# coolbeam/UPFlow_pytorch

Measured on AMD Instinct MI355X. Metric: frame-pairs/sec at 384x1280 bf16, higher is better.
Workload: dtype bf16; 1 GPU; config2: UPFlow_net inference forward (flow fwd+bwd, occlusion masks, SGU on), 384x1280, batch 4 per GPU, random-init weights; global_batch=4, parallelism=replicas x1 (image pairs sharded, no collective), ranks=1, hip_graph=True, capture_fallback=False, steps_in_flight=4, pyramid_convs=HIP (MFMA kernel), pyramid_dtype=fp16

## Files before the change

### include/upflow_hip.h

```cpp
#ifndef UPFLOW_HIP_H
#define UPFLOW_HIP_H

#ifdef __cplusplus
extern "C" {
#endif

enum { UPF_F32 = 0, UPF_F16 = 1, UPF_BF16 = 2 };
enum { UPF_OK = 0, UPF_EINVAL = -1, UPF_EDTYPE = -2, UPF_EALIGN = -3, UPF_EUNSUPPORTED = -4 };
enum { UPF_MASK_NONE = 0, UPF_MASK_LITERAL = 1, UPF_MASK_ROBUST = 2 };

const char* upf_version(void);
const char* upf_last_error(void);

int upf_corr81_forward(const void* f1, const void* f2, void* out,
                       int B, int C, int H, int W, int dtype,
                       long long out_batch_stride, float leaky_slope, void* stream);

int upf_corr81_forward_timed(const void* f1, const void* f2, void* out,
                             int B, int C, int H, int W, int dtype,
                             long long out_batch_stride, float leaky_slope, void* stream,
                             int nrep, float* avg_us, float* min_us);

int upf_corr81_norm_supported(int C, int dtype);
long long upf_corr81_norm_workspace_bytes(int B, int C, int H, int W);
// ... 81 lines not shown

long long upf_conv_packed_bytes(int Cin, int Cout, int kernel_size);
int upf_conv_pack_weights(const void* w , void* w_packed, int Cin, int Cout, int kernel_size,
                          int dtype, void* stream);
int upf_conv_forward(const void* x, long long x_batch_stride, const void* w_packed, const float* bias,
                     void* y, long long y_batch_stride, int B, int Cin, int Cout, int H, int W,
                     int kernel_size, int dilation, int stride, float leaky_slope, int dtype, void* stream);
int upf_conv_forward_pitched(const void* x, long long x_batch_stride, int x_row_pitch, const void* w_packed, const float* bias,
                             void* y, long long y_batch_stride, int y_row_pitch, int B, int Cin, int Cout, int H, int W,
                             int kernel_size, int dilation, int stride, float leaky_slope, int dtype, void* stream);
int upf_conv1x1_forward_mixed(const void* x, long long x_batch_stride, int x_row_pitch, const void* w_packed, const float* bias,
                              void* y, long long y_batch_stride, int y_row_pitch, int y_is_c8, int B, int Cin, int Cout, int H, int W,
                              float leaky_slope, int dtype, int out_dtype, void* stream);
int upf_conv1x1_forward_c8_dual(const void* x, long long x_batch_stride, int x_row_pitch, const void* w_packed, const float* bias,
                                void* y8_a, long long ya_batch_stride, void* y8_b, long long yb_batch_stride,
                                int B, int Cin, int Cout, int H, int W, float leaky_slope, int dtype, int out_dtype, void* stream);
int upf_conv_set_option(const char* name, int value);

long long upf_conv_x3_packed_bytes(int Cin, int Cout, int kernel_size);
int upf_conv_x3_pack_weights(const float* w, void* w_packed, int Cin, int Cout, int kernel_size, void* stream);
int upf_conv_x3_forward(const float* x, long long x_batch_stride, const void* w_packed, const float* bias, float* y,
                        long long y_batch_stride, int B, int Cin, int Cout, int H, int W, int kernel_size, int dilation,
                        int stride, float leaky_slope, int nprod, void* stream);
int upf_conv_x3_set_option(const char* name, int value);
int upf_mfma_f16_denorm_probe(float* out_device, void* stream);

long long upf_conv_packed_bytes_k(int K, int Cout, int kernel_size);
int upf_conv_c8_k(int n8_oct, int C2);
int upf_conv_pack_weights_kmap(const void* w , void* w_packed, int Cin, int Cout, int kernel_size,
                               const int* kmap , int K, int dtype, void* stream);
int upf_conv_forward_c8(const void* x8, long long x8_batch_stride, int n8_oct, const void* x2, long long x2_batch_stride, int C2,
                        const void* w_packed, const float* bias, void* y, long long y_batch_stride, int y_is_c8,
                        int B, int Cout, int H, int W, int kernel_size, int dilation, int stride, float leaky_slope,
                        int dtype, void* stream);
int upf_conv_forward_c8_pitched(const void* x8, long long x8_batch_stride, int n8_oct, const void* x2, long long x2_batch_stride, int x2_row_pitch, int C2,
                                const void* w_packed, const float* bias, void* y, long long y_batch_stride, int y_row_pitch, int y_is_c8,
                                int B, int Cout, int H, int W, int kernel_size, int dilation, int stride, float leaky_slope,
                                int dtype, void* stream);
int upf_conv_c8_set_option(const char* name, int value);
long long upf_conv_packed_bytes_k16(int K, int Cout);
int upf_conv_pack_weights_kmap16(const void* w , void* w_packed, int Cin, int Cout,
                                 const int* kmap , int K, int dtype, void* stream);
int upf_conv_forward_c8_narrow(const void* x8, long long x8_batch_stride, int n8_oct, const void* w_packed16, const float* bias,
                               void* y, long long y_batch_stride, int y_is_c8, int B, int Cout, int H, int W, float leaky_slope,
                               int dtype, void* stream);
int upf_conv_forward_c8_split(const void* x8, long long x8_batch_stride, int n8_oct, const void* w_packed ,
                              const float* bias , void* y8, long long y_batch_stride, int C_main,
                              float* partial, long long partial_batch_stride , int partial_pitch ,
                              int B, int Cout, int H, int W, float leaky_slope, int dtype, void* stream);
int upf_conv_forward_c8_narrow_init(const void* x8, long long x8_batch_stride, int n8_oct, const void* w_packed16,
                                    const float* partial, long long partial_batch_stride, int partial_pitch, int partial_offset ,
                                    void* y, long long y_batch_stride, int y_is_c8, int B, int Cout, int H, int W, float leaky_slope,
                                    int dtype, void* stream);

int upf_conv_pair_forward(const void* x, long long x_batch_stride, int x_row_pitch, int Cin,
                          const void* wa_packed, const float* bias_a , float slope_a, int C1, int stride_a,
                          const void* wb_packed, const float* bias_b , float slope_b, int C2, int stride_b,
                          void* y, long long y_batch_stride, int y_row_pitch, int y_is_c8,
                          int B, int H, int W, int dtype, void* stream);

int upf_conv_pack_weights_f32(const float* w , void* w_packed, int Cin, int Cout, int kernel_size,
                              int dtype, int dgrad, void* stream);
int upf_conv_pack_weights_f32_multi(const float* const* w, void* const* w_packed, const int* Cin, const int* Cout, const int* kernel_size,
                                    const int* dgrad, int njobs, int dtype, void* stream);
int upf_conv_pack_stacked_dgrad(const float* const* w, const int* Cin, const int* Cout, const int* first_channel, int nlayers,
                                void* const* w_packed, const int* slice_channel, const int* slice_width, const int* nconsumers,
                                int nslices, int dtype, void* stream);
int upf_leaky_backward(const void* grad_y, const void* y, void* grad_pre, long long n, float slope, int dtype, void* stream);
int upf_conv_wgrad_supported(int Cin, int Cout, int H, int W, int kernel_size, int dilation, int stride, int dtype);
long long upf_conv_wgrad_workspace_bytes(int B, int Cin, int Cout, int H, int W, int kernel_size, int dilation);
int upf_conv_wgrad(const void* x, long long x_batch_stride, const void* grad_pre, long long g_batch_stride, float* grad_w,
                   void* workspace, int B, int Cin, int Cout, int H, int W, int kernel_size, int dilation, int dtype, void* stream);
typedef struct {
  const void* x;        long long x_batch_stride;
  const void* grad_pre; long long g_batch_stride;
  int B, H, W;
} upf_wgrad_level;
long long upf_conv_wgrad_multi_workspace_bytes(const upf_wgrad_level* levels, int nlevels, int Cin, int Cout, int kernel_size, int dilation);
int upf_conv_wgrad_multi(const upf_wgrad_level* levels , int nlevels, float* grad_w, void* workspace, int Cin, int Cout,
                         int kernel_size, int dilation, int dtype, void* stream);
int upf_conv_wgrad_multi_bias(const upf_wgrad_level* levels, int nlevels, float* grad_w, void* workspace, int Cin, int Cout,
                              int kernel_size, int dilation, const float* const* bias_partials , int npartials, float* grad_bias,
                              int dtype, void* stream);
int upf_space_to_depth2(const void* src, void* dst, int B, int C , int H, int W , int inverse, int dtype, void* stream);
int upf_conv_wgrad_s2d(const upf_wgrad_level* levels, int nlevels, float* grad_w, void* workspace, int Cin, int Cout, int dtype, void* stream);
int upf_act_grad(const void* src, long long src_batch_stride, const void* add, long long add_batch_stride, const void* y,
                 long long y_batch_stride, void* dst, long long dst_batch_stride, float* bias_partial, int B, int C, int HW,
                 float slope, int dtype, void* stream);
int upf_conv_forward_gated(const void* x, long long x_batch_stride, int x_row_pitch, const void* w_packed, const float* bias,
                           void* y, long long y_batch_stride, int y_row_pitch, const void* add, long long add_batch_stride,
                           const void* act, long long act_batch_stride, float mask_slope,
                           int B, int Cin, int Cout, int H, int W, int dtype, void* stream);
int upf_conv_bias_grad_finish(const float* const* partials , int npartials, float* grad_bias,
                              int Cout, void* stream);
long long upf_conv_bias_grad_workspace_bytes(int Cout);
int upf_conv_bias_grad(const void* grad_pre, long long g_batch_stride, float* grad_bias, void* workspace, int B, int Cout, int HW,
                       int dtype, void* stream);

int upf_act_grad_x3(const float* grad_y, long long gy_batch_stride, const float* y, long long y_batch_stride, float* grad_pre_scaled,
                    long long dst_batch_stride, float* bias_partial, float* scale_slot, int B, int C, int HW, float slope, void* stream);
int upf_conv_x3_pack_weights_dgrad(const float* w, void* w_packed, int Cin, int Cout, int kernel_size, void* stream);
int upf_conv_x3_dgrad(const float* grad_pre_scaled, long long g_batch_stride, const float* scale_slot, const float* w,
                      void* w_packed_dgrad, const float* zero_bias, float* grad_x, long long gx_batch_stride, int B, int Cin,
                      int Cout, int H, int W, int kernel_size, int dilation, int stride, void* stream);
int upf_conv_x3_wgrad_workspace_bytes(const upf_wgrad_level* levels, int nlevels, int Cin, int Cout, int kernel_size,
                                      int dilation, int stride, long long* bytes );
// ... 49 lines not shown
```

### upflow_pytorch_amd/_build.py

```python
import os
import subprocess
import sys

PKG = os.path.dirname(os.path.abspath(__file__))
CSRC = os.path.join(PKG, 'csrc')
LIB = os.path.join(PKG, 'libupflow_hip.so')

SOURCES = [
    ('api.hip', []),
    ('corr81_fwd.hip', ['-ffp-contract=off']),
    ('corr81_bwd.hip', []),
    ('conv3x3.hip', []),
    ('conv_c8.hip', []),
    ('conv_pair.hip', []),
    ('conv_x3.hip', []),
    ('conv_x3_bwd.hip', []),
    ('conv_wgrad.hip', []),
    ('warp.hip', ['-ffp-contract=off']),
    ('sgu_blend.hip', ['-ffp-contract=off']),
    ('misc.hip', ['-ffp-contract=off']),
    ('loss.hip', ['-ffp-contract=off']),
]
COMMON = ['--offload-arch=gfx950', '-O3', '-std=c++17', '-fPIC', '-fno-gpu-rdc', '-Wall', '-Wno-unused-function']
NO_PACKED_FP32 = ['-Xclang', '-target-feature', '-Xclang', '-packed-fp32-ops']


def hipcc():
    for c in (os.environ.get('HIPCC'), '/opt/rocm/bin/hipcc', 'hipcc'):
        if c and (os.path.isabs(c) and os.path.exists(c) or not os.path.isabs(c)):
            return c
    raise RuntimeError('hipcc not found')


def _stale(target, deps):
    if not os.path.exists(target):
        return True
    t = os.path.getmtime(target)
    return any(os.path.getmtime(d) > t for d in deps)


def _flags_tag(extra):
    import hashlib
    return hashlib.sha256(' '.join(COMMON + NO_PACKED_FP32 + list(extra)).encode()).hexdigest()[:16]


def _flags_stale(obj, extra):
    try:
        return open(obj + '.flags').read().strip() != _flags_tag(extra)
    except OSError:
        return True


def build(force=False, verbose=False):
    headers = [os.path.join(CSRC, h) for h in os.listdir(CSRC) if h.endswith('.hpp')]
    headers.append(os.path.join(os.path.dirname(PKG), 'include', 'upflow_hip.h'))
    objdir = os.path.join(PKG, 'build')
    os.makedirs(objdir, exist_ok=True)
    objs = []
    cc = hipcc()
    jobs = []
    for src, extra in SOURCES:
        s = os.path.join(CSRC, src)
        o = os.path.join(objdir, src.replace('.hip', '.o'))
        objs.append(o)
        if force or _stale(o, [s] + headers) or _flags_stale(o, extra):
            jobs.append(([cc] + COMMON + NO_PACKED_FP32 + extra + ['-c', s, '-o', o], o, extra))

# ... 29 lines not shown
```

### upflow_pytorch_amd/_lib.py

```python
import ctypes
import os

import torch

_PKG = os.path.dirname(os.path.abspath(__file__))
LIB_PATH = os.environ.get('UPF_HIP_LIB') or os.path.join(_PKG, 'libupflow_hip.so')

UPF_F32, UPF_F16, UPF_BF16 = 0, 1, 2
MASK_NONE, MASK_LITERAL, MASK_ROBUST = 0, 1, 2
_DTYPES = {torch.float32: UPF_F32, torch.float16: UPF_F16, torch.bfloat16: UPF_BF16}

_c = ctypes
_vp, _i, _f, _ll = _c.c_void_p, _c.c_int, _c.c_float, _c.c_longlong

SIGNATURES = {
    'upf_corr81_forward': [_vp, _vp, _vp, _i, _i, _i, _i, _i, _ll, _f, _vp],
    'upf_corr81_forward_timed': [_vp, _vp, _vp, _i, _i, _i, _i, _i, _ll, _f, _vp, _i, _c.POINTER(_f), _c.POINTER(_f)],
    'upf_corr81_norm_forward': [_vp, _vp, _vp, _i, _i, _i, _i, _i, _ll, _f, _vp, _vp],
    'upf_corr81_norm_forward_timed': [_vp, _vp, _vp, _i, _i, _i, _i, _i, _ll, _f, _vp, _vp, _i, _c.POINTER(_f), _c.POINTER(_f)],
    'upf_corr81_norm_forward_c8_timed': [_vp, _vp, _vp, _ll, _i, _i, _i, _i, _i, _f, _vp, _vp, _i, _c.POINTER(_f), _c.POINTER(_f)],
    'upf_corr81_norm_forward_pitched': [_vp, _vp, _i, _vp, _i, _i, _i, _i, _i, _ll, _f, _vp, _vp],
    'upf_corr81_norm_forward_c8_pitched': [_vp, _vp, _i, _vp, _ll, _i, _i, _i, _i, _i, _f, _vp, _vp],
    'upf_corr81_norm_forward_c8_timed_pitched': [_vp, _vp, _i, _vp, _ll, _i, _i, _i, _i, _i, _f, _vp, _vp, _i, _c.POINTER(_f), _c.POINTER(_f)],
    'upf_corr81_norm_forward_c8_timed_mixed': [_vp, _vp, _i, _vp, _ll, _i, _i, _i, _i, _i, _i, _f, _vp, _vp, _i, _c.POINTER(_f), _c.POINTER(_f)],
    'upf_warp_forward_pitched': [_vp, _ll, _i, _vp, _vp, _ll, _i, _i, _i, _i, _i, _i, _i, _i, _vp],
    'upf_conv_forward_gated': [_vp, _ll, _i, _vp, _vp, _vp, _ll, _i, _vp, _ll, _vp, _ll, _f, _i, _i, _i, _i, _i, _i, _vp],
    'upf_conv_forward_pitched': [_vp, _ll, _i, _vp, _vp, _vp, _ll, _i, _i, _i, _i, _i, _i, _i, _i, _i, _f, _i, _vp],
    'upf_conv_forward_c8_pitched': [_vp, _ll, _i, _vp, _ll, _i, _i, _vp, _vp, _vp, _ll, _i, _i, _i, _i, _i, _i, _i, _i, _i, _f, _i, _vp],
    'upf_corr81_norm_forward_mixed': [_vp, _vp, _i, _vp, _i, _i, _i, _i, _i, _i, _ll, _f, _vp, _vp],
    'upf_corr81_norm_forward_c8_mixed': [_vp, _vp, _i, _vp, _ll, _i, _i, _i, _i, _i, _i, _f, _vp, _vp],
    'upf_conv1x1_forward_mixed': [_vp, _ll, _i, _vp, _vp, _vp, _ll, _i, _i, _i, _i, _i, _i, _i, _f, _i, _i, _vp],
    'upf_conv1x1_forward_c8_dual': [_vp, _ll, _i, _vp, _vp, _vp, _ll, _vp, _ll, _i, _i, _i, _i, _i, _f, _i, _i, _vp],
    'upf_corr81_backward': [_vp, _vp, _vp, _vp, _vp, _i, _i, _i, _i, _i, _vp],
    'upf_correlation_forward': [_vp, _vp, _vp, _i, _i, _i, _i, _i, _i, _i, _i, _i, _i, _i, _vp],
    'upf_correlation_backward': [_vp, _vp, _vp, _vp, _vp, _i, _i, _i, _i, _i, _i, _i, _i, _i, _i, _i, _vp],
    'upf_correlation_out_shape': [_i, _i, _i, _i, _i, _i, _i, _c.POINTER(_i), _c.POINTER(_i), _c.POINTER(_i)],
    'upf_warp_forward': [_vp, _vp, _vp, _i, _i, _i, _i, _i, _i, _i, _vp],
    'upf_warp_forward_strided': [_vp, _ll, _vp, _vp, _ll, _i, _i, _i, _i, _i, _i, _i, _vp],
    'upf_warp_forward_c8': [_vp, _ll, _vp, _vp, _ll, _i, _i, _i, _i, _i, _i, _i, _vp],
    'upf_flow_update': [_vp, _vp, _vp, _vp, _ll, _i, _i, _i, _i, _vp],
    'upf_flow_update_c8': [_vp, _vp, _vp, _vp, _ll, _i, _i, _i, _vp],
    'upf_corr81_norm_forward_c8': [_vp, _vp, _vp, _ll, _i, _i, _i, _i, _i, _f, _vp, _vp],
    'upf_warp_backward': [_vp, _vp, _vp, _vp, _vp, _vp, _i, _i, _i, _i, _i, _i, _i, _vp],
    'upf_flow_upsample_forward': [_vp, _vp, _i, _i, _i, _i, _i, _i, _i, _vp],
    'upf_flow_upsample_backward': [_vp, _vp, _i, _i, _i, _i, _i, _i, _i, _vp],
    'upf_sgu_blend_forward': [_vp, _vp, _vp, _vp, _vp, _vp, _i, _i, _i, _i, _i, _i, _vp],
    'upf_sgu_blend_forward_flow16': [_vp, _vp, _vp, _vp, _ll, _i, _i, _i, _i, _i, _vp],
    'upf_sgu_blend_backward': [_vp, _vp, _vp, _vp, _vp, _vp, _i, _i, _i, _i, _i, _i, _vp],
    'upf_normalize_forward': [_vp, _vp, _vp, _vp, _vp, _ll, _i, _i, _vp],
    'upf_normalize_backward': [_vp, _vp, _vp, _vp, _ll, _i, _i, _vp],
    'upf_conv_pack_weights': [_vp, _vp, _i, _i, _i, _i, _vp],
    'upf_conv_forward': [_vp, _ll, _vp, _vp, _vp, _ll, _i, _i, _i, _i, _i, _i, _i, _i, _f, _i, _vp],
    'upf_conv_x3_pack_weights': [_vp, _vp, _i, _i, _i, _vp],
    'upf_conv_x3_forward': [_vp, _ll, _vp, _vp, _vp, _ll, _i, _i, _i, _i, _i, _i, _i, _i, _f, _i, _vp],
    'upf_mfma_f16_denorm_probe': [_vp, _vp],
    'upf_act_grad_x3': [_vp, _ll, _vp, _ll, _vp, _ll, _vp, _vp, _i, _i, _i, _f, _vp],
    'upf_conv_x3_pack_weights_dgrad': [_vp, _vp, _i, _i, _i, _vp],
    'upf_conv_x3_dgrad': [_vp, _ll, _vp, _vp, _vp, _vp, _vp, _ll, _i, _i, _i, _i, _i, _i, _i, _i, _vp],
    'upf_conv_x3_wgrad_workspace_bytes': [_vp, _i, _i, _i, _i, _i, _i, _c.POINTER(_ll)],
    'upf_conv_x3_wgrad': [_vp, _vp, _i, _vp, _vp, _i, _i, _i, _i, _i, _vp, _vp, _vp],
    'upf_conv_pack_weights_f32': [_vp, _vp, _i, _i, _i, _i, _i, _vp],
    'upf_conv_pack_stacked_dgrad': [_c.POINTER(_vp), _c.POINTER(_i), _c.POINTER(_i), _c.POINTER(_i), _i, _c.POINTER(_vp), _c.POINTER(_i), _c.POINTER(_i), _c.POINTER(_i), _i, _i, _vp],
    'upf_conv_pack_weights_f32_multi': [_c.POINTER(_vp), _c.POINTER(_vp), _c.POINTER(_i), _c.POINTER(_i), _c.POINTER(_i), _c.POINTER(_i), _i, _i, _vp],
    'upf_conv_pack_weights_kmap': [_vp, _vp, _i, _i, _i, _vp, _i, _i, _vp],
    'upf_conv_forward_c8': [_vp, _ll, _i, _vp, _ll, _i, _vp, _vp, _vp, _ll, _i, _i, _i, _i, _i, _i, _i, _i, _f, _i, _vp],
    'upf_conv_pack_weights_kmap16': [_vp, _vp, _i, _i, _vp, _i, _i, _vp],
    'upf_conv_forward_c8_narrow': [_vp, _ll, _i, _vp, _vp, _vp, _ll, _i, _i, _i, _i, _i, _f, _i, _vp],
    'upf_conv_forward_c8_split': [_vp, _ll, _i, _vp, _vp, _vp, _ll, _i, _vp, _ll, _i, _i, _i, _i, _i, _f, _i, _vp],
    'upf_conv_forward_c8_narrow_init': [_vp, _ll, _i, _vp, _vp, _ll, _i, _i, _vp, _ll, _i, _i, _i, _i, _i, _f, _i, _vp],
    'upf_conv_pair_forward': [_vp, _ll, _i, _i, _vp, _vp, _f, _i, _i, _vp, _vp, _f, _i, _i, _vp, _ll, _i, _i, _i, _i, _i, _i, _vp],
    'upf_leaky_backward': [_vp, _vp, _vp, _ll, _f, _i, _vp],
    'upf_conv_wgrad': [_vp, _ll, _vp, _ll, _vp, _vp, _i, _i, _i, _i, _i, _i, _i, _i, _vp],
    'upf_conv_bias_grad': [_vp, _ll, _vp, _vp, _i, _i, _i, _i, _vp],
    'upf_conv_wgrad_multi': [_vp, _i, _vp, _vp, _i, _i, _i, _i, _i, _vp],
    'upf_conv_wgrad_multi_bias': [_vp, _i, _vp, _vp, _i, _i, _i, _i, _vp, _i, _vp, _i, _vp],
    'upf_space_to_depth2': [_vp, _vp, _i, _i, _i, _i, _i, _i, _vp],
    'upf_conv_wgrad_s2d': [_vp, _i, _vp, _vp, _i, _i, _i, _vp],
    'upf_act_grad': [_vp, _ll, _vp, _ll, _vp, _ll, _vp, _ll, _vp, _i, _i, _i, _f, _i, _vp],
    'upf_conv_bias_grad_finish': [_vp, _i, _vp, _i, _vp],
    'upf_census_forward': [_vp, _vp, _vp, _i, _i, _i, _i, _vp],
    'upf_census_backward': [_vp, _vp, _vp, _vp, _vp, _i, _i, _i, _i, _vp],
    'upf_boundary_warp_forward': [_vp, _vp, _vp, _vp, _i, _i, _i, _i, _i, _i, _vp],
    'upf_boundary_warp_backward': [_vp, _vp, _vp, _vp, _vp, _i, _i, _i, _i, _i, _i, _vp],
    'upf_robust_loss_forward': [_vp, _vp, _vp, _vp, _i, _i, _i, _f, _f, _vp],
    'upf_robust_loss_backward': [_vp, _vp, _vp, _vp, _vp, _vp, _i, _i, _i, _f, _f, _vp],
    'upf_grey_forward': [_vp, _vp, _i, _i, _vp],
    'upf_msd_upup_forward': [_vp, _vp, _vp, _i, _vp, _vp, _vp, _vp, _i, _i, _i, _f, _f, _f, _vp],
    'upf_msd_upup_backward': [_vp, _vp, _vp, _vp, _i, _vp, _vp, _vp, _vp, _i, _i, _i, _f, _f, _f, _vp],
    'upf_smooth_edge1_forward': [_vp, _vp, _vp, _i, _i, _i, _i, _i, _vp],
    'upf_smooth_edge1_backward': [_vp, _vp, _vp, _vp, _i, _i, _i, _i, _i, _vp],
    'upf_div_selftest': [_i, _vp, _vp],
    'upf_occ_check': [_vp, _vp, _vp, _vp, _i, _i, _i, _f, _f, _vp],
}



class WgradLevel(_c.Structure):
    _fields_ = [('x', _vp), ('x_batch_stride', _ll), ('grad_pre', _vp), ('g_batch_stride', _ll), ('B', _i), ('H', _i), ('W', _i)]


_lib = None


class UpflowHipError(RuntimeError):
    """Raised for a rejected argument or a failed launch (the reference raises RuntimeError through
    AT_ERROR("CUDA call failed"), correlation_cuda.cc:81-83)."""


def lib():
    global _lib
    if _lib is None:
        if not os.path.exists(LIB_PATH):
            raise UpflowHipError(
                '%s is missing: build it with `python -c "import __graft_entry__ as g; g.build()"` '
                '(hipcc --offload-arch=gfx950). There is no CPU fallback.' % LIB_PATH)
        L = ctypes.CDLL(LIB_PATH)
        for name, argtypes in SIGNATURES.items():
            fn = getattr(L, name)
            fn.argtypes = argtypes
            fn.restype = _i
        L.upf_normalize_workspace_bytes.argtypes = [_ll, _i]
        L.upf_normalize_workspace_bytes.restype = _ll
# ... 91 lines not shown
```

### upflow_pytorch_amd/model/pwc_modules.py

```python
import logging

import torch
import torch.nn as nn
import torch.nn.functional as tf

from .. import ops
from ..utils.tools import tools


def conv(in_planes, out_planes, kernel_size=3, stride=1, dilation=1, isReLU=True, if_IN=False, IN_affine=False, if_BN=False):
    layers = [nn.Conv2d(in_planes, out_planes, kernel_size=kernel_size, stride=stride, dilation=dilation,
                        padding=((kernel_size - 1) * dilation) // 2, bias=True)]
    if isReLU:
        layers.append(nn.LeakyReLU(0.1, inplace=True))
    if if_IN:
        layers.append(nn.InstanceNorm2d(out_planes, affine=IN_affine))
    elif if_BN:
        layers.append(nn.BatchNorm2d(out_planes, affine=IN_affine))
    return nn.Sequential(*layers)


def initialize_msra(modules):
    logging.info("Initializing MSRA")
    for layer in modules:
        if isinstance(layer, (nn.Conv2d, nn.ConvTranspose2d)):
            nn.init.kaiming_normal_(layer.weight)
            if layer.bias is not None:
                nn.init.constant_(layer.bias, 0)


def upsample2d_as(inputs, target_as, mode="bilinear"):
    _, _, h, w = target_as.size()
    return tf.interpolate(inputs, [h, w], mode=mode, align_corners=True)


def _resize_flow(inputs, h, w, mode, if_rate):
    if mode != "bilinear":
        res = tf.interpolate(inputs, [h, w], mode=mode)
        if if_rate:
            _, _, h_, w_ = inputs.size()
            scale = torch.tensor([w / w_, h / h_], dtype=res.dtype, device=res.device).view(1, 2, 1, 1)
            res = res * scale
        return res
    return ops.flow_upsample(inputs, h, w, if_rate)


def upsample2d_flow_as(inputs, target_as, mode="bilinear", if_rate=False):
    _, _, h, w = target_as.size()
    return _resize_flow(inputs, h, w, mode, if_rate)


def upsample_flow(inputs, target_size=None, target_flow=None, mode="bilinear"):
    if target_size is not None:
# ... 231 lines not shown
                J.append(j); used += need
            if not J or any(widths[k] % 8 for k in range(m, n - 1)):
                continue
            score = len(J) * (cin[m] + 1000)
            if score > best_score:
                best, best_score = (m, sorted(J)), score
        return best

    def _key(self):
        k = []
        for c in self.convs:
            k += [c.weight._version, c.weight.dtype, c.weight.device, c.weight.data_ptr(), c.bias._version, c.bias.data_ptr()]
        return tuple(k)

    def get(self):
        key = self._key()
        if key != self.key:
            c0 = self.main
            rows, bias = [c0.weight.detach()], [c0.bias.detach().float()]
            self.finish = {}
            for j, c in zip(self.J, self.convs[1:]):
                front = sum(self.widths[self.m:j])
                w = c.weight.detach()
                assert w.shape[1] == front + self.cin
                pad = (c.out_channels + 3) // 4 * 4 - c.out_channels
                rows.append(w[:, front:])
                bias.append(c.bias.detach().float())
                if pad:
                    rows.append(w.new_zeros((pad, self.cin) + tuple(w.shape[2:])))
                    bias.append(bias[0].new_zeros(pad))
                self.finish[j] = ops.conv_c8_pack16(w[:, :front].contiguous(), list(range(front)))
            self.packed = ops.conv_c8_pack(torch.cat(rows, 0).contiguous(), self.kmap)
            self.bias = torch.cat(bias).contiguous()
            self.key = key
        return self.packed, self.bias

    def extra_operands(self):
        return list(self.finish.values())

    def invalidate(self):
        self.key = None

    def main_pass(self, x8, y8):
        packed, bias = self.get()
        B, _, H, W, _ = x8.shape
        part = torch.empty((B, self.pp // 4, H, W, 4), dtype=torch.float32, device=x8.device)
        ops.conv_c8_forward_split_raw(x8, packed, bias, y8, part, self.slopes[self.m])
        return part

    def finish_pass(self, j, x8_front, part, y):
        self.get()
        return ops.conv_c8_forward_narrow_init_raw(x8_front, self.finish[j], part, self.offsets[j], self.widths[j], y, self.slopes[j])


class _PackedConvPair(object):

    def __init__(self, seq_a, seq_b):
        self.convs = (seq_a[0], seq_b[0])
        self.strides = (seq_a[0].stride[0], seq_b[0].stride[0])
        self.slopes = tuple(0.1 if any(isinstance(m_, nn.LeakyReLU) for m_ in q) else 0.0 for q in (seq_a, seq_b))
        self.key = None
        self.packed = self.packed_b = self.bias = self.bias_b = None

    def _key(self):
        k = []
        for c in self.convs:
            k += [c.weight._version, c.weight.dtype, c.weight.device, c.weight.data_ptr(), c.bias._version, c.bias.data_ptr()]
        return tuple(k)

    def get(self):
        key = self._key()
        if key != self.key:
            a, b = self.convs
            self.packed, self.packed_b = ops.conv_pair_pack(a.weight, b.weight)
            self.bias, self.bias_b = a.bias.detach().float().contiguous(), b.bias.detach().float().contiguous()
            self.key = key
        return self.packed, self.bias, self.packed_b, self.bias_b

    def extra_operands(self):
        return [self.packed_b, self.bias_b]

    def invalidate(self):
        self.key = None

    def __call__(self, x, y):
        pa, ba, pb, bb = self.get()
        return ops.conv_pair_forward_raw(x, pa, ba, self.slopes[0], pb, bb, self.slopes[1], y, self.strides)


DUAL_1X1 = [True]
FUSE_PAIRS = [True]
MERGE_TAIL = [True]


def c8_level_ok(nb, H, W, dtype):
    return dtype in (torch.bfloat16, torch.float16) and nb * ((W + 31) // 32) * ((H + 7) // 8) >= 200


def fast_conv_seq(seq, x, cache, out=None, allow_hip=True, pitched=False):
    c = seq[0]
    k = c.kernel_size[0]
    if (allow_hip and _fast_conv_ok(x) and c.kernel_size in ((3, 3), (1, 1)) and c.stride[0] == c.stride[1] and c.groups == 1 and len(seq) <= 2
            and c.padding == (((k - 1) * c.dilation[0]) // 2,) * 2
            and (ops.conv3x3_supported(x, c.out_channels, c.dilation[0], c.stride[0], k)
                 or (x.shape[3] < 8 and 1 <= c.dilation[0] <= 16 and (c.stride[0] == 1 or (c.stride[0] == 2 and c.dilation[0] == 1 and k == 3))))):
        pc = cache.get(id(seq))
        if pc is None:
            pc = cache[id(seq)] = _PackedConv3x3(seq)
        ho, wo = ops.conv3x3_out_hw(x.shape[2], x.shape[3], c.stride[0])
        y = out if out is not None else ops.empty_nchw((x.shape[0], c.out_channels, ho, wo), x.dtype, x.device, pitched=pitched)
        return pc(x, y)
    if torch.is_grad_enabled() and x.is_cuda and x.dtype in (torch.bfloat16, torch.float16) and c.weight.dtype == torch.float32:
        y = train_conv_seq(seq, x)
    elif (FP32_TRAIN_CONV[0] == 'hip_x3' and torch.is_grad_enabled() and x.is_cuda and x.dtype == torch.float32
          and c.weight.dtype == torch.float32):
        y = train_conv_seq_x3(seq, x)
    else:
        y = seq(x if x.is_contiguous() else x.contiguous())
    if out is not None:
        out.copy_(y)
        return out
    return y


def train_conv_seq(seq, x):
    c = seq[0]
    k = c.kernel_size[0]
    slope = 0.0
    for m in list(seq)[1:]:
        if isinstance(m, nn.LeakyReLU):
            slope = float(m.negative_slope)
        else:
            return seq(x.float()).to(x.dtype)
    if (c.kernel_size in ((3, 3), (1, 1)) and c.stride[0] == c.stride[1] and c.groups == 1 and c.padding == (((k - 1) * c.dilation[0]) // 2,) * 2
            and ops.conv_train_supported(x, c.weight, c.stride[0], c.dilation[0])):
        return ops.conv_train(x, c.weight, c.bias, c.dilation[0], slope, c.stride[0])
    return seq(x.float()).to(x.dtype)


def train_conv_seq_x3(seq, x):
    c = seq[0]
    k = c.kernel_size[0]
    slope = 0.0
    for m in list(seq)[1:]:
        if not isinstance(m, nn.LeakyReLU):
# ... 69 lines not shown
        return buf, buf[:, x0:self._n_total]

    def forward_in_buffer(self, buf, out=None):
        if self._packed is None:
            self._packed = [_PackedConv3x3(getattr(self, n)) for n in self._NAMES] + [_PackedConv3x3(self.conv_last)]
        nt = self._n_total
        hi = nt - self._ch_in
        for pc, f in zip(self._packed[:5], self._f):
            pc(buf[:, hi:nt], buf[:, hi - f:hi])
            hi -= f
        x5 = buf[:, :nt]
        if out is None:
            out = torch.empty((buf.shape[0], self.conv_last[0].out_channels) + tuple(buf.shape[2:]), dtype=buf.dtype, device=buf.device)
        self._packed[5](x5, out)
        return x5, out

    def c8_ok(self):
        return self._ch_in % 8 == 0 and all(f % 8 == 0 for f in self._f)

    def c8_outputs_ok(self):
        return all(f % 8 == 0 for f in self._f)

    def forward_in_buffer_c8(self, buf8, out=None, in_map=None):
        key = None if in_map is None else tuple(in_map)
        cache = self.__dict__.setdefault('_packed8', {})
        if key not in cache:
            imap = list(range(self._ch_in)) if in_map is None else list(in_map)
            assert len(imap) % 8 == 0 and sorted(m for m in imap if m >= 0) == list(range(self._ch_in)), 'in_map must place every input channel once'
            packed, nconv = [], 0
            for name, f in zip(self._NAMES, self._f):
                packed.append(_PackedConvC8(getattr(self, name), list(range(nconv)) + [m + nconv if m >= 0 else -1 for m in imap]))
                nconv += f
            packed.append(_PackedConvC8(self.conv_last, list(range(nconv)) + [m + nconv if m >= 0 else -1 for m in imap]))
            widths = list(self._f) + [self.conv_last[0].out_channels]
            seqs = [getattr(self, n_) for n_ in self._NAMES] + [self.conv_last]
            plain = all(all(isinstance(x_, (nn.Conv2d, nn.LeakyReLU)) for x_ in q_) for q_ in seqs)
            pl = _PackedTailC8.plan(widths) if plain else None
            if pl is not None:
                nbefore = sum(self._f[:pl[0]])
                packed.append(_PackedTailC8(seqs, pl[0], pl[1], list(range(nbefore)) + [q + nbefore if q >= 0 else -1 for q in imap]))
            cache[key] = (packed, len(imap) // 8)
        packed, n_in = cache[key]
        nl = len(self._f)
        no = sum(self._f) // 8 + n_in
        starts, hi = [], sum(self._f) // 8
        for f in self._f:
            starts.append(hi)
            hi -= f // 8
        starts.append(hi)
        if out is None:
            out = torch.empty((buf8.shape[0], self.conv_last[0].out_channels) + tuple(buf8.shape[2:4]), dtype=buf8.dtype, device=buf8.device)
        tail = packed[nl + 1] if (len(packed) > nl + 1 and MERGE_TAIL[0] and not getattr(self, '_no_merge_tail', False)) else None
        part = None
        for k in range(nl + 1):
            y = buf8[:, starts[k + 1]:starts[k]] if k < nl else out
            if tail is not None and k == tail.m:
                part = tail.main_pass(buf8[:, starts[k]:no], y)
            elif tail is not None and k in tail.J:
                tail.finish_pass(k, buf8[:, starts[k]:starts[tail.m]], part, y)
            else:
                packed[k](buf8[:, starts[k]:no], None, y)
        return out

    def _train_convs(self):
        seqs = [getattr(self, n) for n in self._NAMES] + [self.conv_last]
        slope = None
        for i, q in enumerate(seqs):
            act = list(q)[1:]
            if i < 5:
                if len(act) != 1 or not isinstance(act[0], nn.LeakyReLU):
                    return None, None
                slope = float(act[0].negative_slope)
            elif act:
                return None, None
        return [q[0] for q in seqs], slope

    def train_in_buffer_ok(self, inputs):
        convs, _ = self._train_convs()
        return convs is not None and not getattr(self, '_no_train_buffer', False) and ops.dense_stack_train_supported(inputs, convs)

    def forward_train(self, inputs, flow_tail=None):
        convs, slope = self._train_convs()
        return ops.dense_stack_train(inputs, convs, slope, flow_tail)

    def forward(self, x):
        if _fast_conv_ok(x):
            buf, slot = self.alloc_buffer(x.shape[0], x.shape[2], x.shape[3], x.dtype, x.device)
            slot.copy_(x)
            return self.forward_in_buffer(buf)
        if self.train_in_buffer_ok([x]):
            buf, out = self.forward_train([x])
            return buf, out
        cache = self.__dict__.setdefault('_fast_cache', {})
        for name in self._NAMES:
            x = torch.cat([fast_conv_seq(getattr(self, name), x, cache), x], dim=1)
        return x, fast_conv_seq(self.conv_last, x, cache)


class FlowEstimatorDense_v2(_DenseStack):
    def __init__(self, ch_in, f_channels=(128, 128, 96, 64, 32), out_channel=2):
        super(FlowEstimatorDense_v2, self).__init__()
        self.n_channels = self._build(ch_in, f_channels, out_channel)


class FlowEstimatorDense(FlowEstimatorDense_v2):

    def __init__(self, ch_in):
        super(FlowEstimatorDense, self).__init__(ch_in)


# ... 51 lines not shown
```

### upflow_pytorch_amd/ops.py

```python
import os

import torch
from torch.autograd import Function

from . import _lib
from ._operand_cache import OperandCache
from ._lib import MASK_NONE, MASK_LITERAL, MASK_ROBUST, UpflowHipError

_MASKS = {None: MASK_NONE, 'none': MASK_NONE, 'literal': MASK_LITERAL, 'robust': MASK_ROBUST,
          MASK_NONE: MASK_NONE, MASK_LITERAL: MASK_LITERAL, MASK_ROBUST: MASK_ROBUST}


def _f32(t):
    return t if t.dtype == torch.float32 else t.float()


PITCH_MULTIPLE = 8


def empty_nchw(shape, dtype, device, pitched=True):
    W = shape[-1]
    if pitched and dtype in (torch.bfloat16, torch.float16) and W >= 8 and W % PITCH_MULTIPLE:
        Wp = (W + PITCH_MULTIPLE - 1) // PITCH_MULTIPLE * PITCH_MULTIPLE
        return torch.empty(tuple(shape[:-1]) + (Wp,), dtype=dtype, device=device)[..., :W]
# ... 746 lines not shown
        if not _c8_view_ok(y) or tuple(y.shape) != (B, (Cout + 7) // 8, H, W, 8):
            raise UpflowHipError('conv_c8_narrow: C8 output must be [%d,%d,%d,%d,8], got %s' % (B, (Cout + 7) // 8, H, W, tuple(y.shape)))
    elif tuple(y.shape) != (B, Cout, H, W) or y.stride()[1:] != (H * W, W, 1):
        raise UpflowHipError('conv_c8_narrow: NCHW output must be a [%d,%d,%d,%d] channel slice' % (B, Cout, H, W))
    dev = x8.device
    if not (x8.is_cuda and y.is_cuda) or x8.dtype != y.dtype:
        raise UpflowHipError('conv_c8_narrow: GPU tensors of one dtype expected (there is no CPU fallback)')
    with torch.cuda.device(dev):
        _lib.call('upf_conv_forward_c8_narrow', _lib.ptr(x8), x8.stride(0), n, _lib.ptr(packed16), _lib.ptr(bias32), _lib.ptr(y), y.stride(0),
                  int(y_is_c8), B, Cout, H, W, float(leaky_slope), _lib.dtype_code(x8), _lib.stream_ptr(dev))
    return y


def _partial_ok(partial, B, H, W):
    return (partial.dtype == torch.float32 and partial.dim() == 5 and partial.shape[0] == B and tuple(partial.shape[2:]) == (H, W, 4)
            and partial.stride()[1:] == (H * W * 4, W * 4, 4, 1))


def conv_c8_forward_split_raw(x8, packed, bias32, y8, partial, leaky_slope=0.0):
    B, n, H, W, _ = x8.shape
    Cout = bias32.shape[0]
    if not _c8_view_ok(x8) or not _c8_view_ok(y8) or tuple(y8.shape[0:1] + y8.shape[2:]) != (B, H, W, 8):
        raise UpflowHipError('conv_c8_split: x8 / y8 must be octet slices of contiguous C8 buffers of one size')
    cmain = 8 * y8.shape[1]
    if not _partial_ok(partial, B, H, W) or 4 * partial.shape[1] < (Cout - cmain + 3) // 4 * 4:
        raise UpflowHipError('conv_c8_split: partial must be fp32 [B,Q,H,W,4] (planes of channel quads, 4 Q >= the partial channels), got %s' % (tuple(partial.shape),))
    dev = x8.device
    if not (x8.is_cuda and y8.is_cuda and partial.is_cuda) or x8.dtype != y8.dtype:
        raise UpflowHipError('conv_c8_split: GPU tensors of one 16-bit dtype expected (there is no CPU fallback)')
    with torch.cuda.device(dev):
        _lib.call('upf_conv_forward_c8_split', _lib.ptr(x8), x8.stride(0), n, _lib.ptr(packed), _lib.ptr(bias32), _lib.ptr(y8), y8.stride(0), cmain,
                  _lib.ptr(partial), partial.stride(0), 4 * partial.shape[1], B, Cout, H, W, float(leaky_slope), _lib.dtype_code(x8), _lib.stream_ptr(dev))
    return y8


def conv_c8_forward_narrow_init_raw(x8, packed16, partial, offset, Cout, y, leaky_slope=0.0):
    B, n, H, W, _ = x8.shape
    y_is_c8 = y.dim() == 5
    if not _c8_view_ok(x8):
        raise UpflowHipError('conv_c8_narrow_init: x8 must be an octet slice of a contiguous C8 buffer')
    if y_is_c8:
        if not _c8_view_ok(y) or tuple(y.shape) != (B, (Cout + 7) // 8, H, W, 8):
            raise UpflowHipError('conv_c8_narrow_init: C8 output must be [%d,%d,%d,%d,8], got %s' % (B, (Cout + 7) // 8, H, W, tuple(y.shape)))
    elif tuple(y.shape) != (B, Cout, H, W) or y.stride()[1:] != (H * W, W, 1):
        raise UpflowHipError('conv_c8_narrow_init: NCHW output must be a [%d,%d,%d,%d] channel slice' % (B, Cout, H, W))
    if not _partial_ok(partial, B, H, W):
        raise UpflowHipError('conv_c8_narrow_init: partial must be fp32 [B,Q,H,W,4] (planes of channel quads)')
    dev = x8.device
    if not (x8.is_cuda and y.is_cuda and partial.is_cuda) or x8.dtype != y.dtype:
        raise UpflowHipError('conv_c8_narrow_init: GPU tensors of one 16-bit dtype expected (there is no CPU fallback)')
    with torch.cuda.device(dev):
        _lib.call('upf_conv_forward_c8_narrow_init', _lib.ptr(x8), x8.stride(0), n, _lib.ptr(packed16), _lib.ptr(partial), partial.stride(0), 4 * partial.shape[1],
                  int(offset), _lib.ptr(y), y.stride(0), int(y_is_c8), B, int(Cout), H, W, float(leaky_slope), _lib.dtype_code(x8), _lib.stream_ptr(dev))
    return y


def conv_pair_pack(w_a, w_b):
    C1, Cin, C2 = w_a.shape[0], w_a.shape[1], w_b.shape[0]
    if tuple(w_a.shape[2:]) != (3, 3) or tuple(w_b.shape[2:]) != (3, 3) or w_b.shape[1] != C1 or Cin > 16 or C1 not in (16, 32) or C2 > 32:
        raise UpflowHipError('conv_pair_pack: 3x3 layers with Cin <= 16, C1 = 16 | 32, C2 <= 32 expected, got %s / %s' % (tuple(w_a.shape), tuple(w_b.shape)))
    dev, dt = w_a.device, w_a.dtype
    lane = torch.arange(64, device=dev)
    co, kg, j = (lane % 32).view(1, 64, 1), (lane // 32).view(1, 64, 1), torch.arange(8, device=dev).view(1, 1, 8)
    wa = torch.zeros((32, 16, 12), dtype=dt, device=dev)
    wa[:C1, :Cin, :9] = w_a.detach().reshape(C1, Cin, 9)
    if Cin <= 4:
        s = torch.arange(3, device=dev).view(3, 1, 1)
        pa = wa[co.expand(3, 64, 8), (j % 4).expand(3, 64, 8), (4 * s + 2 * kg + j // 4).expand(3, 64, 8)]
    elif Cin <= 8:
        s = torch.arange(5, device=dev).view(5, 1, 1)
        pa = wa[co.expand(5, 64, 8), j.expand(5, 64, 8), (2 * s + kg).expand(5, 64, 8)]
    else:
        s = torch.arange(9, device=dev).view(9, 1, 1)
        pa = wa[co.expand(9, 64, 8), (8 * kg + j).expand(9, 64, 8), s.expand(9, 64, 8)]
    ksb = C1 // 16
    wbz = torch.zeros((32, C1, 9), dtype=dt, device=dev)
    wbz[:C2] = w_b.detach().reshape(C2, C1, 9)
    tap = torch.arange(9, device=dev).view(9, 1, 1, 1)
    ks = torch.arange(ksb, device=dev).view(1, ksb, 1, 1)
    shp = (9, ksb, 64, 8)
    pb = wbz[co.view(1, 1, 64, 1).expand(shp), (16 * ks + 8 * kg.view(1, 1, 64, 1) + j.view(1, 1, 1, 8)).expand(shp), tap.expand(shp)]
    return pa.contiguous(), pb.contiguous()


def conv_pair_forward_raw(x, packed_a, bias_a, slope_a, packed_b, bias_b, slope_b, y, strides=(1, 2)):
    B, Cin, H, W = x.shape
    C1, C2 = bias_a.shape[0], bias_b.shape[0]
    Ho, Wo = conv3x3_out_hw(H, W, 2)
    xp = _pitch_or_raise(x, 'conv_pair: x')
    y_is_c8 = y.dim() == 5
    if y_is_c8:
        if not _c8_view_ok(y) or tuple(y.shape) != (B, (C2 + 7) // 8, Ho, Wo, 8):
            raise UpflowHipError('conv_pair: C8 output must be [%d,%d,%d,%d,8], got %s' % (B, (C2 + 7) // 8, Ho, Wo, tuple(y.shape)))
        yp = 0
    else:
        if tuple(y.shape) != (B, C2, Ho, Wo):
            raise UpflowHipError('conv_pair: NCHW output must be [%d,%d,%d,%d], got %s' % (B, C2, Ho, Wo, tuple(y.shape)))
        yp = _out_pitch_or_raise(y, 'conv_pair: y')
    dev = x.device
    if not (x.is_cuda and y.is_cuda) or x.dtype != y.dtype or x.dtype not in (torch.bfloat16, torch.float16) or packed_a.dtype != x.dtype:
        raise UpflowHipError('conv_pair: GPU tensors of one 16-bit dtype expected (there is no CPU fallback)')
    with torch.cuda.device(dev):
        _lib.call('upf_conv_pair_forward', _lib.ptr(x), x.stride(0), xp, Cin, _lib.ptr(packed_a), _lib.ptr(bias_a), float(slope_a), C1, int(strides[0]),
                  _lib.ptr(packed_b), _lib.ptr(bias_b), float(slope_b), C2, int(strides[1]), _lib.ptr(y), y.stride(0), yp, int(y_is_c8), B, H, W,
                  _lib.dtype_code(x), _lib.stream_ptr(dev))
    return y
# ... 1074 lines not shown
```

Baseline: 1943 frame-pairs/s.

## Fuse last two narrow tail convolutions into one kernel with LDS halo recompute

Adds a HIP kernel that runs the final 16->8 conv and the last 8->Cout conv of the dense-net tail in one launch. The intermediate 8-channel activation is computed with a one-pixel halo into LDS and consumed directly by the second conv, while still being written to the C8 buffer. The goal is to save one kernel launch and the global round trip of the middle activation, at the cost of recomputing the halo and using more LDS per block. It is enabled by default when the layer widths match and can be turned off with an environment variable.

```diff
diff --git a/include/upflow_hip.h b/include/upflow_hip.h
--- a/include/upflow_hip.h
+++ b/include/upflow_hip.h
@@ -157,6 +157,10 @@
                                     const float* partial, long long partial_batch_stride, int partial_pitch, int partial_offset ,
                                     void* y, long long y_batch_stride, int y_is_c8, int B, int Cout, int H, int W, float leaky_slope,
                                     int dtype, void* stream);
+int upf_conv_forward_c8_tail2(const void* x8, long long x8_batch_stride, int n8_oct, const void* w_packed16_a, const void* w_packed16_b,
+                              const float* partial, long long partial_batch_stride, int partial_pitch, int partial_offset_a, int partial_offset_b,
+                              void* y_mid8, long long y_mid_batch_stride, int C_mid, void* y, long long y_batch_stride,
+                              int B, int Cout, int H, int W, float leaky_slope_a, float leaky_slope_b, int dtype, void* stream);
 
 int upf_conv_pair_forward(const void* x, long long x_batch_stride, int x_row_pitch, int Cin,
                           const void* wa_packed, const float* bias_a , float slope_a, int C1, int stride_a,
diff --git a/upflow_pytorch_amd/_build.py b/upflow_pytorch_amd/_build.py
--- a/upflow_pytorch_amd/_build.py
+++ b/upflow_pytorch_amd/_build.py
@@ -13,6 +13,7 @@
     ('conv3x3.hip', []),
     ('conv_c8.hip', []),
     ('conv_pair.hip', []),
+    ('conv_tail2.hip', []),
     ('conv_x3.hip', []),
     ('conv_x3_bwd.hip', []),
     ('conv_wgrad.hip', []),
diff --git a/upflow_pytorch_amd/_lib.py b/upflow_pytorch_amd/_lib.py
--- a/upflow_pytorch_amd/_lib.py
+++ b/upflow_pytorch_amd/_lib.py
@@ -68,6 +68,7 @@
     'upf_conv_forward_c8_narrow': [_vp, _ll, _i, _vp, _vp, _vp, _ll, _i, _i, _i, _i, _i, _f, _i, _vp],
     'upf_conv_forward_c8_split': [_vp, _ll, _i, _vp, _vp, _vp, _ll, _i, _vp, _ll, _i, _i, _i, _i, _i, _f, _i, _vp],
     'upf_conv_forward_c8_narrow_init': [_vp, _ll, _i, _vp, _vp, _ll, _i, _i, _vp, _ll, _i, _i, _i, _i, _i, _f, _i, _vp],
+    'upf_conv_forward_c8_tail2': [_vp, _ll, _i, _vp, _vp, _vp, _ll, _i, _i, _i, _vp, _ll, _i, _vp, _ll, _i, _i, _i, _i, _f, _f, _i, _vp],
     'upf_conv_pair_forward': [_vp, _ll, _i, _i, _vp, _vp, _f, _i, _i, _vp, _vp, _f, _i, _i, _vp, _ll, _i, _i, _i, _i, _i, _i, _vp],
     'upf_leaky_backward': [_vp, _vp, _vp, _ll, _f, _i, _vp],
     'upf_conv_wgrad': [_vp, _ll, _vp, _ll, _vp, _vp, _i, _i, _i, _i, _i, _i, _i, _i, _vp],
diff --git a/upflow_pytorch_amd/csrc/conv_tail2.hip b/upflow_pytorch_amd/csrc/conv_tail2.hip
--- /dev/null
+++ b/upflow_pytorch_amd/csrc/conv_tail2.hip
@@ -0,0 +1,212 @@
+#include "conv_kernel.hpp"
+
+namespace upf {
+namespace conv {
+
+struct Tail2Part { const float* part; long long pbs; int ppitch, coffa, coffb; };
+
+template <typename T, int RPW>
+__global__ __launch_bounds__(NTHREADS, 4)
+void conv_tail2_sgu_kernel(const T* __restrict__ x8, long long x8bs, const T* __restrict__ wpa, const T* __restrict__ wpb,
+                           T* __restrict__ ymid, long long ymbs, T* __restrict__ y, long long ybs, int CoutB, int H, int W,
+                           int tiles_x, int tiles_y, float slope_a, float slope_b, const Tail2Part pa) {
+  constexpr int TH = 4 * RPW;
+  constexpr int XR = TH + 4, XC = TW + 4, XP = XC | 1;
+  constexpr int MR = TH + 2, MC = TW + 2, MP = MC | 1;
+  constexpr int EB = 2 * XR * XP, EBP = (EB + 63) & ~63, NSL = (EBP / 64 + 3) / 4;
+  constexpr int NPX = MR * MC, NG = (NPX + 15) / 16, NGW = (NG + 3) / 4;
+  extern __shared__ __attribute__((aligned(16))) uint4 xs[];
+  uint4* mid = xs + EBP;
+
+  const int bid = xcd_remap(blockIdx.x, gridDim.x);
+  const int tx = bid % tiles_x, ty = (bid / tiles_x) % tiles_y, n = bid / (tiles_x * tiles_y);
+  const int x0 = tx * TW, y0 = ty * TH;
+  const int tid = threadIdx.x, lane = tid & 63;
+  const int wave_u = __builtin_amdgcn_readfirstlane(tid >> 6);
+  const int p16 = lane & 15, ko = lane >> 4;
+  const int HW = H * W;
+
+  __amdgpu_buffer_rsrc_t x8r = __builtin_amdgcn_make_buffer_rsrc(const_cast<T*>(x8 + (size_t)n * x8bs), 0, 2u * (uint32_t)HW * 16u, 0x00020000);
+#pragma unroll
+  for (int j = 0; j < NSL; ++j) {
+    const int piece = j * 4 + wave_u;
+    if (piece * 64 < EBP) {
+      const int p = piece * 64 + lane;
+      const int oct = p / (XR * XP), rem = p - oct * (XR * XP), r = rem / XP, col = rem - r * XP;
+      const int gy = y0 - 2 + r, gx = x0 - 2 + col;
+      const bool in = p < EB && col < XC && gy >= 0 && gy < H && gx >= 0 && gx < W;
+      const uint32_t voff = in ? (uint32_t)((oct * HW + gy * W + gx) * 16) : 0x80000000u;
+      __builtin_amdgcn_raw_ptr_buffer_load_lds(x8r, (__attribute__((address_space(3))) void*)(xs + piece * 64), 16, (int)voff, 0, 0, 0);
+    }
+  }
+
+  __amdgpu_buffer_rsrc_t pr = __builtin_amdgcn_make_buffer_rsrc(const_cast<float*>(pa.part + (size_t)n * pa.pbs), 0, (uint32_t)HW * (uint32_t)pa.ppitch * 4u, 0x00020000);
+  f32x4 acca[NGW];
+#pragma unroll
+  for (int i = 0; i < NGW; ++i) {
+    const int q = (wave_u + 4 * i) * 16 + p16, qq = q < NPX ? q : 0;
+    const int mr = qq / MC, mc = qq - mr * MC, gy = y0 - 1 + mr, gx = x0 - 1 + mc;
+    const bool in = q < NPX && gy >= 0 && gy < H && gx >= 0 && gx < W && ko < 2;
+    const uint32_t off = in ? (uint32_t)(((pa.coffa >> 2) + ko) * HW + gy * W + gx) * 16u : 0x80000000u;
+    acca[i] = __builtin_bit_cast(f32x4, __builtin_amdgcn_raw_buffer_load_b128(pr, off, 0, 0));
+  }
+
+  uint4 wa[9];
+#pragma unroll
+  for (int tap = 0; tap < 9; ++tap) wa[tap] = reinterpret_cast<const uint4*>(wpa)[tap * 64 + lane];
+
+  asm volatile("s_waitcnt vmcnt(0)" ::: "memory");
+  __syncthreads();
+
+  __amdgpu_buffer_rsrc_t mr_ = __builtin_amdgcn_make_buffer_rsrc(ymid + (size_t)n * ymbs, 0, (uint32_t)HW * 16u, 0x00020000);
+  __builtin_amdgcn_s_setprio(2);
+#pragma unroll
+  for (int i = 0; i < NGW; ++i) {
+    if (wave_u + 4 * i < NG) {
+      const int q = (wave_u + 4 * i) * 16 + p16, qq = q < NPX ? q : 0;
+      const int mr = qq / MC, mc = qq - mr * MC, gy = y0 - 1 + mr, gx = x0 - 1 + mc;
+      const bool in = q < NPX && gy >= 0 && gy < H && gx >= 0 && gx < W;
+      const uint4* xb = xs + ((ko & 1) * XR + mr) * XP + mc;
+      uint4 b[9];
+#pragma unroll
+      for (int tap = 0; tap < 9; ++tap) {
+        b[tap] = xb[(tap / 3) * XP + tap % 3];
+        if (ko >= 2) b[tap] = make_uint4(0u, 0u, 0u, 0u);
+      }
+      f32x4 acc = acca[i];
+#pragma unroll
+      for (int tap = 0; tap < 9; ++tap) acc = Mma16<T>::mma(wa[tap], b[tap], acc);
+      float v[4];
+#pragma unroll
+      for (int k = 0; k < 4; ++k) { v[k] = acc[k]; v[k] = fmaxf(v[k], v[k] * slope_a); }
+      u32x2 o;
+      o.x = pack2<T>(v[0], v[1]); o.y = pack2<T>(v[2], v[3]);
+      if (!in) { o.x = 0u; o.y = 0u; }
+      if (q < NPX && ko < 2) reinterpret_cast<u32x2*>(mid)[(mr * MP + mc) * 2 + ko] = o;
+      const bool own = in && ko < 2 && mr >= 1 && mr <= TH && mc >= 1 && mc <= TW;
+      __builtin_amdgcn_raw_buffer_store_b64(o, mr_, own ? (uint32_t)(gy * W + gx) * 16u + (uint32_t)ko * 8u : 0x80000000u, 0, 0);
+    }
+  }
+  __builtin_amdgcn_s_setprio(0);
+  const int rg = wave_u;
+  f32x4 accb[RPW][2];
+#pragma unroll
+  for (int r = 0; r < RPW; ++r)
+#pragma unroll
+    for (int h = 0; h < 2; ++h) {
+      const int gx = x0 + p16 + 16 * h, gy = y0 + RPW * rg + r;
+      const uint32_t off = (gx < W && gy < H && 4 * ko < CoutB) ? (uint32_t)(((pa.coffb >> 2) + ko) * HW + gy * W + gx) * 16u : 0x80000000u;
+      accb[r][h] = __builtin_bit_cast(f32x4, __builtin_amdgcn_raw_buffer_load_b128(pr, off, 0, 0));
+    }
+  uint4 wb[9];
+#pragma unroll
+  for (int tap = 0; tap < 9; ++tap) wb[tap] = reinterpret_cast<const uint4*>(wpb)[tap * 64 + lane];
+  __syncthreads();
+
+  constexpr int NR = RPW + 2;
+  const uint4* bb = ko == 0 ? mid + (RPW * rg) * MP + p16 : xs + (((ko - 1) & 1) * XR + RPW * rg + 1) * XP + p16 + 1;
+  const int bp = ko == 0 ? MP : XP;
+  uint4 bq[2][6];
+  auto bload = [&](int sr, uint4 (&b)[6]) {
+#pragma unroll
+    for (int h = 0; h < 2; ++h)
+#pragma unroll
+      for (int kx = 0; kx < 3; ++kx) {
+        b[h * 3 + kx] = bb[sr * bp + 16 * h + kx];
+        if (ko == 3) b[h * 3 + kx] = make_uint4(0u, 0u, 0u, 0u);
+      }
+  };
+  __builtin_amdgcn_s_setprio(2);
+  bload(0, bq[0]);
+#pragma unroll
+  for (int sr = 0; sr < NR; ++sr) {
+    if (sr + 1 < NR) bload(sr + 1, bq[(sr + 1) & 1]);
+    __builtin_amdgcn_sched_barrier(0);
+#pragma unroll
+    for (int kx = 0; kx < 3; ++kx)
+#pragma unroll
+      for (int h = 0; h < 2; ++h)
+#pragma unroll
+        for (int ky = 0; ky < 3; ++ky)
+          if (sr - ky >= 0 && sr - ky < RPW)
+            accb[sr - ky][h] = Mma16<T>::mma(wb[ky * 3 + kx], bq[sr & 1][h * 3 + kx], accb[sr - ky][h]);
+    __builtin_amdgcn_sched_barrier(0);
+  }
+  __builtin_amdgcn_s_setprio(0);
+
+  const uint32_t plane2 = (uint32_t)HW * 2u;
+  __amdgpu_buffer_rsrc_t yr = __builtin_amdgcn_make_buffer_rsrc(y + (size_t)n * ybs, 0, (uint32_t)CoutB * plane2, 0x00020000);
+#pragma unroll
+  for (int r = 0; r < RPW; ++r) {
+    const int gy = y0 + RPW * rg + r;
+    if (gy < H) {
+#pragma unroll
+      for (int h = 0; h < 2; ++h) {
+        const int gx = x0 + p16 + 16 * h;
+        float v[4];
+#pragma unroll
+        for (int k = 0; k < 4; ++k) { v[k] = accb[r][h][k]; v[k] = fmaxf(v[k], v[k] * slope_b); }
+        const uint32_t off = (gx < W) ? (uint32_t)(4 * ko) * plane2 + (uint32_t)(gy * W + gx) * 2u : 0x80000000u;
+        const uint32_t p01 = pack2<T>(v[0], v[1]), p23 = pack2<T>(v[2], v[3]);
+        __builtin_amdgcn_raw_buffer_store_b16((unsigned short)p01, yr, off, 0, 0);
+        __builtin_amdgcn_raw_buffer_store_b16((unsigned short)(p01 >> 16), yr, off + plane2, 0, 0);
+        __builtin_amdgcn_raw_buffer_store_b16((unsigned short)p23, yr, off + 2u * plane2, 0, 0);
+        __builtin_amdgcn_raw_buffer_store_b16((unsigned short)(p23 >> 16), yr, off + 3u * plane2, 0, 0);
+      }
+    }
+  }
+}
+
+struct ArgsTail2 {
+  const void* x8; long long x8bs; const void* wpa; const void* wpb; void* ymid; long long ymbs; void* y; long long ybs;
+  int B, CoutB, H, W; float slope_a, slope_b; hipStream_t stream;
+};
+
+template <typename T, int RPW>
+int launch_tail2_sgu(const ArgsTail2& a, const Tail2Part& pa) {
+  constexpr int TH = 4 * RPW;
+  constexpr int EB = 2 * (TH + 4) * ((TW + 4) | 1), EBP = (EB + 63) & ~63;
+  const int tiles_x = cdiv(a.W, TW), tiles_y = cdiv(a.H, TH);
+  const size_t lds = (size_t)(EBP + (TH + 2) * ((TW + 2) | 1)) * 16;
+  static LdsOptIn opt;
+  auto kern = &conv_tail2_sgu_kernel<T, RPW>;
+  opt.ensure(reinterpret_cast<const void*>(kern), lds);
+  hipLaunchKernelGGL(kern, dim3((unsigned)(a.B * tiles_x * tiles_y)), dim3(NTHREADS), lds, a.stream, (const T*)a.x8, a.x8bs, (const T*)a.wpa, (const T*)a.wpb,
+                     (T*)a.ymid, a.ymbs, (T*)a.y, a.ybs, a.CoutB, a.H, a.W, tiles_x, tiles_y, a.slope_a, a.slope_b, pa);
+  return check_launch("conv_forward_c8_tail2");
+}
+
+
+}
+}
+
+extern "C" int upf_conv_forward_c8_tail2(const void* x8, long long x8_batch_stride, int n8_oct, const void* w_packed16_a, const void* w_packed16_b,
+                                         const float* partial, long long partial_batch_stride, int partial_pitch, int partial_offset_a, int partial_offset_b,
+                                         void* y_mid8, long long y_mid_batch_stride, int C_mid, void* y, long long y_batch_stride,
+                                         int B, int Cout, int H, int W, float leaky_slope_a, float leaky_slope_b, int dtype, void* stream) {
+  using namespace upf;
+  UPF_REQUIRE(x8 && w_packed16_a && w_packed16_b && partial && y_mid8 && y, UPF_EINVAL, "conv_forward_c8_tail2: null pointer");
+  UPF_REQUIRE(n8_oct == 2 && C_mid == 8, UPF_EUNSUPPORTED, "conv_forward_c8_tail2: a 16 -> 8 first layer only (got %d octets -> %d channels)", n8_oct, C_mid);
+  UPF_REQUIRE(B > 0 && Cout > 0 && Cout <= 16 && H > 0 && W > 0, UPF_EINVAL, "conv_forward_c8_tail2: bad shape B=%d Cout=%d (<= 16) H=%d W=%d", B, Cout, H, W);
+  UPF_REQUIRE(partial_pitch % 4 == 0 && partial_offset_a % 4 == 0 && partial_offset_a >= 0 && partial_offset_a + C_mid <= partial_pitch &&
+              partial_offset_b % 4 == 0 && partial_offset_b >= 0 && partial_offset_b + (Cout + 3) / 4 * 4 <= partial_pitch, UPF_EINVAL,
+              "conv_forward_c8_tail2: partial pitch %d / offsets %d, %d must be multiples of 4 floats holding the layers' %d and %d channels",
+              partial_pitch, partial_offset_a, partial_offset_b, C_mid, Cout);
+  UPF_REQUIRE(dtype == UPF_BF16 || dtype == UPF_F16, UPF_EDTYPE, "conv_forward_c8_tail2: bf16 / fp16 only");
+  UPF_REQUIRE(aligned_to(x8, 16) && x8_batch_stride % 8 == 0 && aligned_to(partial, 16) && partial_batch_stride % 4 == 0, UPF_EINVAL,
+              "conv_forward_c8_tail2: the C8 input and the partial must be 16-byte aligned");
+  UPF_REQUIRE(aligned_to(y_mid8, 16) && y_mid_batch_stride % 8 == 0, UPF_EINVAL, "conv_forward_c8_tail2: the C8 output must be 16-byte aligned");
+  UPF_REQUIRE(aligned_to(w_packed16_a, 16) && aligned_to(w_packed16_b, 16), UPF_EINVAL, "conv_forward_c8_tail2: the packed operands must be 16-byte aligned");
+  UPF_REQUIRE((long long)n8_oct * H * W * 16 < (1ll << 31) && (long long)H * W * partial_pitch * 4 < (1ll << 31), UPF_EINVAL,
+              "conv_forward_c8_tail2: image too large for one buffer descriptor");
+  UPF_REQUIRE((long long)Cout * H * W * 2 < (1ll << 31), UPF_EINVAL, "conv_forward_c8_tail2: output too large for one buffer descriptor");
+  UPF_REQUIRE(leaky_slope_a >= 0.f && leaky_slope_a <= 1.f && leaky_slope_b >= 0.f && leaky_slope_b <= 1.f, UPF_EINVAL,
+              "conv_forward_c8_tail2: leaky slopes %g, %g not in [0,1]", (double)leaky_slope_a, (double)leaky_slope_b);
+  const conv::ArgsTail2 a{x8, x8_batch_stride, w_packed16_a, w_packed16_b, y_mid8, y_mid_batch_stride, y, y_batch_stride, B, Cout, H, W,
+                          leaky_slope_a == 0.f ? 1.f : leaky_slope_a, leaky_slope_b == 0.f ? 1.f : leaky_slope_b, (hipStream_t)stream};
+  const conv::Tail2Part pa{partial, partial_batch_stride, partial_pitch, partial_offset_a, partial_offset_b};
+#define UPF_TAIL2(T) return conv::launch_tail2_sgu<T, 2>(a, pa);
+  if (dtype == UPF_BF16) { UPF_TAIL2(bf16_t) }
+  UPF_TAIL2(f16_t)
+#undef UPF_TAIL2
+}
diff --git a/upflow_pytorch_amd/model/pwc_modules.py b/upflow_pytorch_amd/model/pwc_modules.py
--- a/upflow_pytorch_amd/model/pwc_modules.py
+++ b/upflow_pytorch_amd/model/pwc_modules.py
@@ -1,4 +1,5 @@
 import logging
+import os
 
 import torch
 import torch.nn as nn
@@ -336,6 +337,17 @@
         self.get()
         return ops.conv_c8_forward_narrow_init_raw(x8_front, self.finish[j], part, self.offsets[j], self.widths[j], y, self.slopes[j])
 
+    def pair_ok(self):
+        n = len(self.widths)
+        return (self.J == [n - 2, n - 1] and self.m == n - 3
+                and ops.conv_c8_tail2_supported(self.widths[self.m], self.widths[n - 2], self.widths[n - 1]))
+
+    def finish_pair(self, x8_main, part, y_mid8, y):
+        self.get()
+        ja, jb = self.J
+        return ops.conv_c8_forward_tail2_raw(x8_main, self.finish[ja], self.finish[jb], part, self.offsets[ja], self.offsets[jb], y_mid8,
+                                             self.widths[jb], y, self.slopes[ja], self.slopes[jb])
+
 
 class _PackedConvPair(object):
 
@@ -375,6 +387,7 @@
 DUAL_1X1 = [True]
 FUSE_PAIRS = [True]
 MERGE_TAIL = [True]
+FUSE_TAIL2 = [not os.environ.get('UPF_NO_FUSE_TAIL2')]
 
 
 def c8_level_ok(nb, H, W, dtype):
@@ -550,10 +563,14 @@
             out = torch.empty((buf8.shape[0], self.conv_last[0].out_channels) + tuple(buf8.shape[2:4]), dtype=buf8.dtype, device=buf8.device)
         tail = packed[nl + 1] if (len(packed) > nl + 1 and MERGE_TAIL[0] and not getattr(self, '_no_merge_tail', False)) else None
         part = None
+        pair = tail is not None and FUSE_TAIL2[0] and not getattr(self, '_no_fuse_tail2', False) and tail.pair_ok()
         for k in range(nl + 1):
             y = buf8[:, starts[k + 1]:starts[k]] if k < nl else out
             if tail is not None and k == tail.m:
                 part = tail.main_pass(buf8[:, starts[k]:no], y)
+            elif pair and k in tail.J:
+                if k == nl:
+                    tail.finish_pair(buf8[:, starts[tail.m + 1]:starts[tail.m]], part, buf8[:, starts[nl]:starts[nl - 1]], y)
             elif tail is not None and k in tail.J:
                 tail.finish_pass(k, buf8[:, starts[k]:starts[tail.m]], part, y)
             else:
diff --git a/upflow_pytorch_amd/ops.py b/upflow_pytorch_amd/ops.py
--- a/upflow_pytorch_amd/ops.py
+++ b/upflow_pytorch_amd/ops.py
@@ -822,6 +822,28 @@
     with torch.cuda.device(dev):
         _lib.call('upf_conv_forward_c8_narrow_init', _lib.ptr(x8), x8.stride(0), n, _lib.ptr(packed16), _lib.ptr(partial), partial.stride(0), 4 * partial.shape[1],
                   int(offset), _lib.ptr(y), y.stride(0), int(y_is_c8), B, int(Cout), H, W, float(leaky_slope), _lib.dtype_code(x8), _lib.stream_ptr(dev))
+    return y
+
+
+def conv_c8_tail2_supported(front_a, width_a, width_b):
+    return front_a == 16 and width_a == 8 and 0 < width_b <= 16
+
+
+def conv_c8_forward_tail2_raw(x8, packed16_a, packed16_b, partial, offset_a, offset_b, y_mid8, Cout, y, slope_a=0.0, slope_b=0.0):
+    B, n, H, W, _ = x8.shape
+    if not _c8_view_ok(x8) or not _c8_view_ok(y_mid8) or tuple(y_mid8.shape) != (B, 1, H, W, 8):
+        raise UpflowHipError('conv_c8_tail2: x8 / y_mid8 must be octet slices [%d,n,%d,%d,8] / [%d,1,%d,%d,8] of contiguous C8 buffers' % (B, H, W, B, H, W))
+    if tuple(y.shape) != (B, Cout, H, W) or y.stride()[1:] != (H * W, W, 1):
+        raise UpflowHipError('conv_c8_tail2: NCHW output must be a [%d,%d,%d,%d] channel slice' % (B, Cout, H, W))
+    if not _partial_ok(partial, B, H, W):
+        raise UpflowHipError('conv_c8_tail2: partial must be fp32 [B,Q,H,W,4] (planes of channel quads)')
+    dev = x8.device
+    if not (x8.is_cuda and y.is_cuda and y_mid8.is_cuda and partial.is_cuda) or x8.dtype != y.dtype or x8.dtype != y_mid8.dtype:
+        raise UpflowHipError('conv_c8_tail2: GPU tensors of one 16-bit dtype expected (there is no CPU fallback)')
+    with torch.cuda.device(dev):
+        _lib.call('upf_conv_forward_c8_tail2', _lib.ptr(x8), x8.stride(0), n, _lib.ptr(packed16_a), _lib.ptr(packed16_b), _lib.ptr(partial), partial.stride(0),
+                  4 * partial.shape[1], int(offset_a), int(offset_b), _lib.ptr(y_mid8), y_mid8.stride(0), 8 * y_mid8.shape[1], _lib.ptr(y), y.stride(0),
+                  B, int(Cout), H, W, float(slope_a), float(slope_b), _lib.dtype_code(x8), _lib.stream_ptr(dev))
     return y
 
 
```

Result: no change. 1948 frame-pairs/s (median of 4 runs) (+0.2%).
